# libshoal/Green-Marl

Measured on AMD Instinct MI355X. Metric: edges/s (GTEPS) per PageRank iter, RMAT-26, higher is better.
Workload: dtype f32; 1 GPU; pagerank RMAT-26 (V=67108864, E=1073741824), reference RMAT generator seed 1997 permute=1, d=0.85, fixed iterations; partition=1-D vertex, 1 rank(s), exchange=none, exchange_bytes_per_rank_and_step=0, exchange_packed=False, step_form=single rank, options=15

## Files before the change

### green-marl_amd/csrc/gmx_pr_cold.hip

```cpp
#pragma clang fp contract(off)

#include "gmx_internal.h"

#include <algorithm>
#include <rocprim/rocprim.hpp>

#define PRC_G 32
#define PRC_BLK_GROUPS 16
#define PRC_LDS_BYTES 131072
#define PRC_STAGE_BYTES 2048
#define PRC_LDS_LIMIT 163840
static constexpr int prc_tile_elems(int elem) { return (PRC_LDS_LIMIT - 16 * (PRC_STAGE_BYTES + 64 * elem) - 64) / elem; }
static constexpr int prc_tile_elems_classed(int elem) {
    return (PRC_LDS_LIMIT - 16 * 64 * elem - 64) / elem < 32768 ? (PRC_LDS_LIMIT - 16 * 64 * elem - 64) / elem / 8 * 8 : 32768;
}
#define PRC_THREADS 1024
#define PRC_WAVES (PRC_THREADS / 64)
#define PRC_UNROLL 4
#define PRC_PAD 0xffffu
#define PRC_END 0x8000u
#define PRC_Q1P 0
#define PRC_Q1E 64
#define PRC_Q2 128

#ifdef GMX_PR_BOUNDS
#define PRC_CHECK(cond) do { if (!(cond)) __builtin_trap(); } while (0)
#else
#define PRC_CHECK(cond) do { } while (0)
#endif

#define PRC_CLS_BITS 3
enum { PRC_CL_GEN = 0, PRC_CL_E1 = 1, PRC_CL_E2 = 2, PRC_CL_E4 = 3, PRC_CL_E8 = 4, PRC_CL_H = 5 };
enum { PRC_FORM_EDGE = 0, PRC_FORM_PAIR = 1, PRC_FORM_E1 = 2, PRC_FORM_E2 = 3, PRC_FORM_E4 = 4, PRC_FORM_E8 = 5, PRC_FORM_H = 6,
       PRC_FORM_TILE = 7 };
enum { PRC_TM_EDGE = 0, PRC_TM_PAIR = 1, PRC_TM_CLASSED = 2, PRC_TM_SINGLES = 3 };
__host__ __device__ static inline int prc_class_of_len(int len) { return len <= 1 ? PRC_CL_E1 : len == 2 ? PRC_CL_E2 : len <= 4 ? PRC_CL_E4 : len <= 8 ? PRC_CL_E8 : PRC_CL_H; }
__host__ __device__ static inline int prc_padded_len(int cls, int len) {
    return cls == PRC_CL_GEN ? len : cls == PRC_CL_H ? (len + 7) & ~7 : 1 << (cls - 1);
}

__host__ __device__ static inline int prc_e_stores(int L, int elem) { return ((8 / L) * elem + 15) / 16; }
__host__ __device__ static inline int64_t prc_interleaved_pos(int L, int elem, int64_t G, int i, int j) {
    const int K = prc_e_stores(L, elem), R = 16 / elem, cpg = K / 2;
    const int ch = i / (8 * R), within = i % (8 * R), m = within / R, r = within % R, q = (int) (G & 1) * cpg + ch;
    return (G & ~(int64_t) 1) * PRC_G + 8 * m + (q * R + r) * L + j;
}

struct prc_item1 { int32_t tile, g0, g1, form; };
struct prc_item2 { int32_t bin, g0, g1, slot; };
struct prc_item3 { int32_t bin, slot0, nslots, pad; };

struct pr_cold {
    pr_cold_params prm;
    int64_t Ec = 0;
    int64_t P1 = 0;
    int64_t P2 = 0;
    int64_t npairs = 0;
    int64_t ncold = 0;
    int tile = 0, binrows = 0, limbs = 1, lo_bits = 42;
    int64_t ntiles = 0, nbins = 0, ncells = 0;
    dbuf<uint16_t> srcl;
    dbuf<int32_t> ob;
    dbuf<uint16_t> rowl;
    dbuf<char> val;
    dbuf<char> cold;
    dbuf<prc_item1> it1p;
    dbuf<int32_t> torg;
    dbuf<int32_t> vstart;
    dbuf<prc_item2> it2;
    dbuf<prc_item3> it3;
    int64_t n1p = 0, n1e = 0, n2 = 0, n3 = 0, nslots = 0;
    std::vector<prc_item1> h1p, h1e;
    std::vector<prc_item2> h2;
    std::vector<prc_item3> h3;
    int nparts = 1;
    int64_t o1[3] = {0, 0, 0};
    int64_t o1g[2] = {0, 0};
    std::vector<int64_t> o2, o3, o3few;
    uint32_t q1 = 0, q1c = 0, q2 = 0;
    dbuf<unsigned long long> scratch;
    dbuf<unsigned int> queue;
    dbuf<double> diffp;
    int grid = 256;
    bool all_bins = false;
    std::vector<int32_t> tile_maxdeg;
};

static int prc_grid_for(int64_t n, int block = 256) {
    int64_t b = (n + block - 1) / block;
    if (b < 1) b = 1;
    if (b > 256 * 16) b = 256 * 16;
    return (int) b;
}

__global__ void prc_keys_kernel(const uint64_t* __restrict__ keys, int64_t n, pr_cold_params prm, int tile_src, int binrows,
                                int binbits, uint64_t* __restrict__ out) {
    int64_t i = (int64_t) blockIdx.x * blockDim.x + threadIdx.x;
    const int64_t stride = (int64_t) gridDim.x * blockDim.x;
    const int64_t span = prm.slice - prm.T;
    for (; i < n; i += stride) {
        const uint64_t k = keys[i];
        const int64_t row = (int64_t) (k >> 32) - prm.row_lo;
        const int64_t src = (int64_t) (uint32_t) k;
        const int64_t a = prm.index_of_row[row];
        const int64_t cp = (src / prm.slice) * span + (src % prm.slice - prm.T);
        const uint64_t t = (uint64_t) (cp / tile_src), sl = (uint64_t) (cp % tile_src);
        const uint64_t b = (uint64_t) (a / binrows), rl = (uint64_t) (a % binrows);
        out[i] = (t << (32 + binbits + PRC_CLS_BITS)) | (b << 32) | (rl << 16) | sl;
    }
}

__global__ void prc_runs_kernel(const uint64_t* __restrict__ k, int64_t n, const uint8_t* __restrict__ single, int tshift,
                                int32_t* __restrict__ cflag, int32_t* __restrict__ ps) {
    int64_t i = (int64_t) blockIdx.x * blockDim.x + threadIdx.x;
    const int64_t stride = (int64_t) gridDim.x * blockDim.x;
    for (; i < n; i += stride) {
        cflag[i] = (i == 0 || (k[i] >> 32) != (k[i - 1] >> 32)) ? 1 : 0;
        ps[i] = (i == 0 || (k[i] >> 16) != (k[i - 1] >> 16) || (single && single[k[i] >> tshift] == PRC_TM_SINGLES)) ? 1 : 0;
    }
}

__global__ void prc_pair_start_kernel(const int32_t* __restrict__ ps, const int32_t* __restrict__ pincl, int64_t n, int64_t np,
                                      int32_t* __restrict__ pstart) {
    int64_t i = (int64_t) blockIdx.x * blockDim.x + threadIdx.x;
    const int64_t stride = (int64_t) gridDim.x * blockDim.x;
    for (; i <= n; i += stride) {
        if (i == n) { pstart[np] = (int32_t) n; continue; }
        if (ps[i]) pstart[pincl[i] - 1] = (int32_t) i;
    }
}

__global__ void prc_tile_stats_kernel(const uint64_t* __restrict__ k, int64_t n, int shift, int64_t ntiles, const int32_t* __restrict__ pincl,
                                      const int32_t* __restrict__ cincl, int64_t np, int64_t nc, int32_t* __restrict__ out) {
    int64_t t = (int64_t) blockIdx.x * blockDim.x + threadIdx.x;
    const int64_t stride = (int64_t) gridDim.x * blockDim.x;
    for (; t <= ntiles; t += stride) {
        int64_t lo = 0, hi = n;
        while (lo < hi) {
            const int64_t mid = (lo + hi) >> 1;
            if ((int64_t) (k[mid] >> shift) < t) lo = mid + 1; else hi = mid;
        }
        out[3 * t + 0] = (int32_t) lo;
        out[3 * t + 1] = lo < n ? pincl[lo] - 1 : (int32_t) np;
        out[3 * t + 2] = lo < n ? cincl[lo] - 1 : (int32_t) nc;
    }
}

__global__ void prc_class_kernel(uint64_t* __restrict__ k, int64_t n, const int32_t* __restrict__ pincl, const int32_t* __restrict__ pstart,
                                 const uint8_t* __restrict__ mode, int binbits) {
    int64_t i = (int64_t) blockIdx.x * blockDim.x + threadIdx.x;
    const int64_t stride = (int64_t) gridDim.x * blockDim.x;
    for (; i < n; i += stride) {
        const uint64_t key = k[i];
        const int m = mode[key >> (32 + binbits + PRC_CLS_BITS)];
        if (m == PRC_TM_SINGLES) { k[i] = key | ((uint64_t) PRC_CL_E1 << (32 + binbits)); continue; }
        if (m != PRC_TM_CLASSED) continue;
        const int32_t p = pincl[i] - 1;
// ... 557 lines not shown

template <typename S, int FORM>
__device__ __forceinline__ void prc_class_block(const S* __restrict__ s_tile, S* __restrict__ stage, const prc_u32x4 cur, const int32_t o,
                                                S* __restrict__ val, const unsigned sink, const int lane) {
    if constexpr (FORM == PRC_FORM_H) prc_block_H<S>(s_tile, stage, cur, o, val, sink, lane);
    else prc_block_E<S, 1 << (FORM - PRC_FORM_E1)>(s_tile, cur, o, val, lane);
}

#define PRC_SET_WAIT_N(t, N)                                                                                        \
    asm volatile("s_waitcnt vmcnt(%8)"                                                                              \
                 : "+v"((t).e0), "+v"((t).e1), "+v"((t).e2), "+v"((t).e3), "+v"((t).o0), "+v"((t).o1), "+v"((t).o2), "+v"((t).o3) \
                 : "n"(N) : "memory")

template <typename S, int FORM>
__device__ __forceinline__ void prc_class_item(const prc_item1 d, const S* __restrict__ s_tile, S* __restrict__ stage,
                                               const uint16_t* __restrict__ srcl, const int32_t* __restrict__ ob,
                                               S* __restrict__ val, const unsigned sink, const int wv, const int lane) {
    constexpr int NST = prc_form_stores<S, FORM>::value;
    const int nblocks = (d.g1 - d.g0) / PRC_BLK_GROUPS;
    const int nsuper = nblocks / (PRC_WAVES * PRC_PAIR_DEPTH);
    const prc_u32x4* in = (const prc_u32x4*) srcl + ((int64_t) d.g0 * (PRC_G / 8) + wv * 64 + lane);
    const int32_t* obp = ob + (d.g0 + wv * PRC_BLK_GROUPS + (lane >> 2));
    constexpr int64_t IN_STEP = PRC_PAIR_DEPTH * PRC_WAVES * 64;
    constexpr int64_t OB_STEP = PRC_PAIR_DEPTH * PRC_WAVES * PRC_BLK_GROUPS;
    if (nsuper > 0) {
        prc_set A, B;
#define PRC_PROCESS(t)                                                                  \
    do {                                                                                \
        prc_class_block<S, FORM>(s_tile, stage, (t).e0, (t).o0, val, sink, lane);       \
        prc_class_block<S, FORM>(s_tile, stage, (t).e1, (t).o1, val, sink, lane);       \
        prc_class_block<S, FORM>(s_tile, stage, (t).e2, (t).o2, val, sink, lane);       \
        prc_class_block<S, FORM>(s_tile, stage, (t).e3, (t).o3, val, sink, lane);       \
    } while (0)
        prc_set_load(A, in, obp);
        {
            const int kn = 1 < nsuper ? 1 : 0;
            prc_set_load(B, in + kn * IN_STEP, obp + kn * OB_STEP);
        }
        PRC_SET_WAIT_N(A, 8);
        PRC_PROCESS(A);
        int k = 1;
#pragma unroll 1
        for (; k + 1 < nsuper; k += 2) {
            prc_set_load(A, in + (int64_t) (k + 1) * IN_STEP, obp + (int64_t) (k + 1) * OB_STEP);
            PRC_SET_WAIT_N(B, 4 * NST + 8);
            PRC_PROCESS(B);
            const int kn = k + 2 < nsuper ? k + 2 : k + 1;
            prc_set_load(B, in + (int64_t) kn * IN_STEP, obp + (int64_t) kn * OB_STEP);
            PRC_SET_WAIT_N(A, 4 * NST + 8);
            PRC_PROCESS(A);
        }
        PRC_SET_WAIT_N(B, 4 * NST);
        if (k < nsuper) PRC_PROCESS(B);
#undef PRC_PROCESS
    }
    {
        const int b0 = nsuper * (PRC_WAVES * PRC_PAIR_DEPTH);
        prc_u32x4 cur[PRC_PAIR_DEPTH];
        int32_t o[PRC_PAIR_DEPTH];
#pragma unroll
        for (int j = 0; j < PRC_PAIR_DEPTH; j++)
            if (b0 + j * PRC_WAVES + wv < nblocks) {
                const int64_t off = (int64_t) (b0 + j * PRC_WAVES);
                cur[j] = __builtin_nontemporal_load(in + off * 64);
                o[j] = __builtin_nontemporal_load(obp + off * PRC_BLK_GROUPS);
            }
#pragma unroll
        for (int j = 0; j < PRC_PAIR_DEPTH; j++)
            if (b0 + j * PRC_WAVES + wv < nblocks) prc_class_block<S, FORM>(s_tile, stage, cur[j], o[j], val, sink, lane);
    }
}

template <typename S>
__device__ __forceinline__ void prc_edge_item(const prc_item1 d, const S* __restrict__ s_tile,
                                              const uint16_t* __restrict__ srcl, const int32_t* __restrict__ ob,
                                              S* __restrict__ val, const int wv, const int lane) {
    typedef typename prc_vec4<S>::type V4;
    const int npieces = (d.g1 - d.g0 + 7) >> 3;
    for (int base = 0; base < npieces; base += PRC_WAVES * PRC_UNROLL) {
        prc_u32x2 ids[PRC_UNROLL];
        int32_t o[PRC_UNROLL];
#pragma unroll
        for (int u = 0; u < PRC_UNROLL; u++) {
            const int pc = base + u * PRC_WAVES + wv;
            const int g = d.g0 + pc * 8 + (lane >> 3);
            o[u] = -1;
            if (pc < npieces && g < d.g1) {
                ids[u] = __builtin_nontemporal_load((const prc_u32x2*) srcl + (int64_t) g * (PRC_G / 4) + (lane & 7));
                o[u] = __builtin_nontemporal_load(ob + g);
            }
        }
#pragma unroll
        for (int u = 0; u < PRC_UNROLL; u++) {
            if (o[u] < 0) continue;
            V4 v;
            v.x = s_tile[ids[u].x & 0x7fffu];
            v.y = s_tile[(ids[u].x >> 16) & 0x7fffu];
            v.z = s_tile[ids[u].y & 0x7fffu];
            v.w = s_tile[(ids[u].y >> 16) & 0x7fffu];
            __builtin_nontemporal_store(v, (V4*) (val + o[u]) + (lane & 7));
        }
    }
}

template <typename S, int TILE, bool CLASSED>
__global__ void __launch_bounds__(PRC_THREADS)
pr_cold_tile_kernel(const prc_item1* __restrict__ items, int n_items, unsigned int* __restrict__ queue,
                    const S* __restrict__ contrib, const int32_t* __restrict__ org, int nranks, int64_t span, int64_t slice, int64_t T,
                    const uint16_t* __restrict__ srcl, const int32_t* __restrict__ ob, S* __restrict__ val, unsigned sink_base,
                    unsigned qbase, const int32_t* __restrict__ vst) {
    __shared__ S s_tile[TILE];
    __shared__ S s_stage[PRC_WAVES][CLASSED ? 64 : PRC_STAGE_BYTES / sizeof(S) + 64];
    __shared__ int s_item;
    const int tid = threadIdx.x, lane = tid & 63;
    const int wv = __builtin_amdgcn_readfirstlane(tid >> 6);
    const unsigned sink = sink_base + (blockIdx.x * PRC_WAVES + wv) * 64 + lane;
    int loaded = -1;
    for (;;) {
        __syncthreads();
        if (tid == 0) s_item = (int) (atomicAdd(&queue[CLASSED ? PRC_Q1E : PRC_Q1P], 1u) - qbase);
        __syncthreads();
        const int it = s_item;
        if ((unsigned) it >= (unsigned) n_items) break;
        const prc_item1 d = items[it];
        if (d.tile != loaded) {
            prc_load_tile<S, TILE>(s_tile, d.tile, org, contrib, nranks, span, slice, T);
            loaded = d.tile;
            __syncthreads();
        }
        if constexpr (CLASSED) {
            const int32_t* vs = vst + ((int64_t) d.tile << PRC_CLS_BITS);
            for (int cls = PRC_CL_E1; cls <= PRC_CL_H; cls++) {
                const int32_t lo = max(d.g0, vs[cls]), hi = min(d.g1, vs[cls + 1]);
                if (lo >= hi) continue;
                const prc_item1 seg{d.tile, lo, hi, cls + 1};
                switch (cls) {
                case PRC_CL_E1: prc_class_item<S, PRC_FORM_E1>(seg, s_tile, s_stage[wv], srcl, ob, val, sink, wv, lane); break;
                case PRC_CL_E2: prc_class_item<S, PRC_FORM_E2>(seg, s_tile, s_stage[wv], srcl, ob, val, sink, wv, lane); break;
                case PRC_CL_E4: prc_class_item<S, PRC_FORM_E4>(seg, s_tile, s_stage[wv], srcl, ob, val, sink, wv, lane); break;
                case PRC_CL_E8: prc_class_item<S, PRC_FORM_E8>(seg, s_tile, s_stage[wv], srcl, ob, val, sink, wv, lane); break;
                default: prc_class_item<S, PRC_FORM_H>(seg, s_tile, s_stage[wv], srcl, ob, val, sink, wv, lane); break;
                }
            }
        } else {
            if (d.form == PRC_FORM_PAIR) prc_pair_item<S>(d, s_tile, s_stage[wv], srcl, ob, val, sink, wv, lane);
            else prc_edge_item<S>(d, s_tile, srcl, ob, val, wv, lane);
        }
    }
}

__device__ __forceinline__ unsigned long long prc_fix_hi(double v) { return (unsigned long long) (long long) (v * 0x1p62); }

template <typename S>
__device__ __forceinline__ void prc_finish_row(const pr_cold_fuse& fz, int64_t i, double sum, double& diff_acc) {
    const int32_t od = __builtin_nontemporal_load(fz.outdeg_c + i);
    const int64_t r = __builtin_nontemporal_load(fz.active + i);
    const double old = (double) __builtin_nontemporal_load((const S*) fz.rk_c + i);
    const S vs = (S) (fz.base + fz.d * sum);
    diff_acc += fabs((double) vs - old);
    __builtin_nontemporal_store(vs, (S*) fz.rk_c + i);
    __builtin_nontemporal_store(od > 0 ? (S) ((double) vs / (double) od) : (S) 0, (S*) fz.next_owned + r);
}

template <int THREADS>
__device__ __forceinline__ void prc_block_diff(double diff_acc, double* s_red, double* __restrict__ dst) {
#pragma unroll
    for (int off = 32; off > 0; off >>= 1) diff_acc += __shfl_down(diff_acc, off, 64);
    if ((threadIdx.x & 63) == 0) s_red[threadIdx.x >> 6] = diff_acc;
    __syncthreads();
    if (threadIdx.x == 0) {
        double t = 0.0;
#pragma unroll
        for (int w = 0; w < THREADS / 64; w++) t += s_red[w];
        *dst = t;
    }
}

template <typename S, int BINROWS, int LIMBS, bool FUSE>
__global__ void __launch_bounds__(PRC_THREADS)
pr_cold_accum_kernel(const prc_item2* __restrict__ items, int n_items, unsigned int* __restrict__ queue,
                     const uint16_t* __restrict__ rowl, const S* __restrict__ val, int64_t nactive, double lo_scale,
                     S* __restrict__ cold, unsigned long long* __restrict__ scratch, pr_cold_fuse fz,
                     double* __restrict__ diff_part, unsigned qbase) {
    typedef typename prc_vec4<S>::type V4;
    __shared__ unsigned long long s_acc[LIMBS * BINROWS];
    __shared__ double s_red[PRC_WAVES];
    __shared__ int s_item;
    const int tid = threadIdx.x, lane = tid & 63;
    const int wv = __builtin_amdgcn_readfirstlane(tid >> 6);
    for (;;) {
        __syncthreads();
        if (tid == 0) s_item = (int) (atomicAdd(&queue[PRC_Q2], 1u) - qbase);
#pragma unroll 4
        for (int i = tid; i < LIMBS * BINROWS; i += PRC_THREADS) s_acc[i] = 0ull;
        __syncthreads();
        const int it = s_item;
        if ((unsigned) it >= (unsigned) n_items) break;
        const prc_item2 d = items[it];
        const int npieces = (d.g1 - d.g0 + 7) >> 3;
        for (int base = 0; base < npieces; base += PRC_WAVES * PRC_UNROLL) {
            prc_u32x2 ids[PRC_UNROLL];
            V4 v[PRC_UNROLL];
            bool ok[PRC_UNROLL];
#pragma unroll
            for (int u = 0; u < PRC_UNROLL; u++) {
                const int pc = base + u * PRC_WAVES + wv;
                const int g = d.g0 + pc * 8 + (lane >> 3);
                ok[u] = pc < npieces && g < d.g1;
                if (ok[u]) {
                    const int64_t at = (int64_t) g * (PRC_G / 4) + (lane & 7);
                    ids[u] = __builtin_nontemporal_load((const prc_u32x2*) rowl + at);
                    v[u] = __builtin_nontemporal_load((const V4*) val + at);
                }
            }
#pragma unroll
            for (int u = 0; u < PRC_UNROLL; u++) {
                if (!ok[u]) continue;
                const unsigned r[4] = {ids[u].x & 0xffffu, ids[u].x >> 16, ids[u].y & 0xffffu, ids[u].y >> 16};
                const double x[4] = {(double) v[u].x, (double) v[u].y, (double) v[u].z, (double) v[u].w};
#pragma unroll
                for (int j = 0; j < 4; j++) {
                    if (r[j] == PRC_PAD) continue;
                    PRC_CHECK(r[j] < (unsigned) BINROWS && x[j] >= 0.0 && x[j] <= 1.0);
                    const unsigned long long hi = prc_fix_hi(x[j]);
                    __hip_atomic_fetch_add(&s_acc[r[j]], hi, __ATOMIC_RELAXED, __HIP_MEMORY_SCOPE_WORKGROUP);
                    if (LIMBS > 1) {
                        const double rem = x[j] - (double) (long long) hi * 0x1p-62;
                        const unsigned long long lo = (unsigned long long) (long long) (rem * 0x1p62 * lo_scale);
                        __hip_atomic_fetch_add(&s_acc[BINROWS + r[j]], lo, __ATOMIC_RELAXED, __HIP_MEMORY_SCOPE_WORKGROUP);
                    }
                }
            }
        }
        __syncthreads();
        double diff_acc = 0.0;
        if (d.slot < 0) {
            const int64_t i0 = (int64_t) d.bin * BINROWS;
#pragma unroll 4
            for (int r = tid; r < BINROWS; r += PRC_THREADS) {
                if (i0 + r >= nactive) break;
                double sum = (double) (long long) s_acc[r] * 0x1p-62;
                if (LIMBS > 1) sum += (double) (long long) s_acc[BINROWS + r] * (0x1p-62 / lo_scale);
                if (FUSE) prc_finish_row<S>(fz, i0 + r, sum, diff_acc);
                else __builtin_nontemporal_store((S) sum, cold + i0 + r);
            }
        } else {
            unsigned long long* dst = scratch + (int64_t) d.slot * (LIMBS * BINROWS);
#pragma unroll 4
            for (int i = tid; i < LIMBS * BINROWS; i += PRC_THREADS) dst[i] = s_acc[i];
        }
        if (FUSE) prc_block_diff<PRC_THREADS>(diff_acc, s_red, diff_part + it);
    }
}

template <typename S, int BINROWS, int LIMBS, bool FUSE>
__global__ void __launch_bounds__(1024)
pr_cold_reduce_kernel(const prc_item3* __restrict__ items, int64_t nactive, double lo_scale,
                      const unsigned long long* __restrict__ scratch, S* __restrict__ cold, pr_cold_fuse fz,
                      double* __restrict__ diff_part) {
    __shared__ unsigned long long s_part[LIMBS][16][64];
    const prc_item3 d = items[blockIdx.y];
    const int lane = threadIdx.x & 63, wv = threadIdx.x >> 6;
    const int r = blockIdx.x * 64 + lane;
    const int64_t i0 = (int64_t) d.bin * BINROWS;
    unsigned long long hi = 0, lo = 0;
    const unsigned long long* src = scratch + (int64_t) d.slot0 * (LIMBS * BINROWS) + r;
#pragma unroll 4
    for (int s = wv; s < d.nslots; s += 16) {
        hi += __builtin_nontemporal_load(src + (int64_t) s * (LIMBS * BINROWS));
        if (LIMBS > 1) lo += __builtin_nontemporal_load(src + (int64_t) s * (LIMBS * BINROWS) + BINROWS);
    }
    s_part[0][wv][lane] = hi;
    if (LIMBS > 1) s_part[LIMBS - 1][wv][lane] = lo;
    __syncthreads();
    if (wv == 0 && i0 + r < nactive) {
        hi = 0;
        lo = 0;
#pragma unroll
        for (int w = 0; w < 16; w++) {
            hi += s_part[0][w][lane];
            if (LIMBS > 1) lo += s_part[LIMBS - 1][w][lane];
        }
        double v = (double) (long long) hi * 0x1p-62;
        if (LIMBS > 1) v += (double) (long long) lo * (0x1p-62 / lo_scale);
        if (FUSE) {
            double diff_acc = 0.0;
            prc_finish_row<S>(fz, i0 + r, v, diff_acc);
            s_part[0][0][lane] = (unsigned long long) __double_as_longlong(diff_acc);
        } else cold[i0 + r] = (S) v;
    } else if (FUSE && wv == 0) s_part[0][0][lane] = 0ull;
    if (FUSE && wv == 0) {
        __builtin_amdgcn_wave_barrier();
        __builtin_amdgcn_s_waitcnt(0xc07f);
        __builtin_amdgcn_wave_barrier();
        if (lane == 0) {
            double t = 0.0;
            for (int l = 0; l < 64; l++) t += __longlong_as_double((long long) s_part[0][0][l]);
            diff_part[(int64_t) blockIdx.y * gridDim.x + blockIdx.x] = t;
        }
    }
}

#define PRC_FEW_SLOTS 8
template <typename S, int BINROWS, int LIMBS, bool FUSE>
__global__ void __launch_bounds__(256)
pr_cold_reduce_few_kernel(const prc_item3* __restrict__ items, int64_t nactive, double lo_scale,
                          const unsigned long long* __restrict__ scratch, S* __restrict__ cold, pr_cold_fuse fz,
                          double* __restrict__ diff_part) {
    const prc_item3 d = items[blockIdx.y];
    const int lane = threadIdx.x & 63;
    const int rg = blockIdx.x * 4 + (threadIdx.x >> 6);
    const int r = rg * 64 + lane;
    const int64_t i0 = (int64_t) d.bin * BINROWS;
    unsigned long long hi = 0, lo = 0;
    const unsigned long long* src = scratch + (int64_t) d.slot0 * (LIMBS * BINROWS) + r;
#pragma unroll 4
    for (int s = 0; s < d.nslots; s++) {
        hi += __builtin_nontemporal_load(src + (int64_t) s * (LIMBS * BINROWS));
        if (LIMBS > 1) lo += __builtin_nontemporal_load(src + (int64_t) s * (LIMBS * BINROWS) + BINROWS);
    }
    double diff_acc = 0.0;
    if (i0 + r < nactive) {
        double v = (double) (long long) hi * 0x1p-62;
        if (LIMBS > 1) v += (double) (long long) lo * (0x1p-62 / lo_scale);
        if (FUSE) prc_finish_row<S>(fz, i0 + r, v, diff_acc);
        else cold[i0 + r] = (S) v;
    }
    if (FUSE) {
        double t = 0.0;
        for (int l = 0; l < 64; l++) t += __shfl(diff_acc, l, 64);
        if (lane == 0) diff_part[(int64_t) blockIdx.y * (BINROWS / 64) + rg] = t;
    }
}

static int prc_upload_lists(pr_cold* c, const std::vector<uint8_t>* tile_class, const std::vector<int32_t>* bin_part, int nparts) {
    auto by_size1 = [](const prc_item1& a, const prc_item1& b) { return a.g1 - a.g0 > b.g1 - b.g0; };
    auto by_size2 = [](const prc_item2& a, const prc_item2& b) { return a.g1 - a.g0 > b.g1 - b.g0; };
    std::vector<prc_item1> l1;
    for (int k = 0; k < 2; k++) {
        c->o1[k] = (int64_t) l1.size();
        for (int part = 0; part < 3; part++) {
            if (part == 1) c->o1g[k] = (int64_t) l1.size();
            std::vector<prc_item1> a;
            for (const prc_item1& it : (part < 2 ? c->h1p : c->h1e))
                if ((tile_class ? (int) (*tile_class)[(size_t) it.tile] : 0) == k && (part == 2 || (part == 0) == (it.form >= PRC_FORM_E1))) a.push_back(it);
            std::stable_sort(a.begin(), a.end(), by_size1);
            l1.insert(l1.end(), a.begin(), a.end());
        }
    }
    c->o1[2] = (int64_t) l1.size();
    std::vector<prc_item2> l2;
    std::vector<prc_item3> l3;
    c->o2.assign((size_t) nparts + 1, 0);
    c->o3.assign((size_t) nparts + 1, 0);
    c->o3few.assign((size_t) nparts, 0);
    for (int q = 0; q < nparts; q++) {
        c->o2[(size_t) q] = (int64_t) l2.size();
        c->o3[(size_t) q] = (int64_t) l3.size();
        std::vector<prc_item2> a;
        for (const prc_item2& it : c->h2)
            if ((bin_part ? (*bin_part)[(size_t) it.bin] : 0) == q) a.push_back(it);
        std::stable_sort(a.begin(), a.end(), by_size2);
        l2.insert(l2.end(), a.begin(), a.end());
        for (int few = 1; few >= 0; few--)
            for (const prc_item3& it : c->h3)
                if ((bin_part ? (*bin_part)[(size_t) it.bin] : 0) == q && (it.nslots <= PRC_FEW_SLOTS ? 1 : 0) == few) {
                    l3.push_back(it);
                    if (few) c->o3few[(size_t) q]++;
                }
    }
    c->o2[(size_t) nparts] = (int64_t) l2.size();
    c->o3[(size_t) nparts] = (int64_t) l3.size();
    c->nparts = nparts;
    if ((int64_t) l1.size() != c->n1p + c->n1e || (int64_t) l2.size() != c->n2 || (int64_t) l3.size() != c->n3) {
        gmx_set_error("pr cold: work lists lost items while being regrouped");
        return GMX_ERR_ARG;
    }
    if (!l1.empty()) GMX_HIP(hipMemcpy(c->it1p.p, l1.data(), sizeof(prc_item1) * l1.size(), hipMemcpyHostToDevice));
    if (!l2.empty()) GMX_HIP(hipMemcpy(c->it2.p, l2.data(), sizeof(prc_item2) * l2.size(), hipMemcpyHostToDevice));
    if (!l3.empty()) GMX_HIP(hipMemcpy(c->it3.p, l3.data(), sizeof(prc_item3) * l3.size(), hipMemcpyHostToDevice));
    return GMX_OK;
}

int pr_cold_set_parts(pr_cold* c, int nparts, const int64_t* act_bound, int64_t hub, int64_t live) {
    if (!c || c->Ec == 0) return GMX_OK;
    if (nparts <= 1) return prc_upload_lists(c, nullptr, nullptr, 1);
    std::vector<int32_t> bin_part((size_t) c->nbins, 0);
    {
        std::vector<int64_t> bb((size_t) nparts + 1, 0);
        for (int j = 1; j < nparts; j++) bb[(size_t) j] = std::min<int64_t>(c->nbins, act_bound[j] / c->binrows);
        bb[(size_t) nparts] = c->nbins;
        for (int j = 0; j < nparts; j++)
            for (int64_t b = bb[(size_t) j]; b < bb[(size_t) j + 1]; b++) bin_part[(size_t) b] = nparts - 1 - j;
    }
    std::vector<uint8_t> tile_class((size_t) c->ntiles, 0);
    const int64_t span = c->prm.slice - c->prm.T, tile_src = c->tile - 1;
    for (int64_t t = 0; t < c->ntiles; t++) {
        const int64_t cp0 = t * tile_src, cp1 = std::min<int64_t>(cp0 + tile_src, span * c->prm.nranks);
        bool hub_only = true;
        for (int64_t r = cp0 / span; r * span < cp1 && hub_only; r++) {
            const int64_t o0 = c->prm.T + std::max<int64_t>(cp0, r * span) - r * span;
            const int64_t o1 = c->prm.T + std::min<int64_t>(cp1, (r + 1) * span) - r * span;
            if (o0 < live && std::min(o1, live) > hub) hub_only = false;
        }
// ... 517 lines not shown
```

Before: 748.9 GTEPS.

## Prefetch next work item and vectorize fused row finish in cold accumulate kernel

Restructures the cold accumulate kernel so the first batch of the next queue item is loaded while the current item's rows are finalized, and zeroes shared accumulators inline instead of in a separate pass. The row finish now reads outdegree and old rank as 4-wide vectors. The next-contribution values are staged in LDS so the scatter to next_owned is coalesced by lane. This aims to hide global load latency across item boundaries and cut per-row scalar memory traffic, at the cost of more registers and extra synchronization.

```diff
diff --git a/green-marl_amd/csrc/gmx_pr_cold.hip b/green-marl_amd/csrc/gmx_pr_cold.hip
--- a/green-marl_amd/csrc/gmx_pr_cold.hip
+++ b/green-marl_amd/csrc/gmx_pr_cold.hip
@@ -3,6 +3,7 @@
 #include "gmx_internal.h"
 
 #include <algorithm>
+#include <type_traits>
 #include <rocprim/rocprim.hpp>
 
 #define PRC_G 32
@@ -866,14 +867,19 @@
 __device__ __forceinline__ unsigned long long prc_fix_hi(double v) { return (unsigned long long) (long long) (v * 0x1p62); }
 
 template <typename S>
+__device__ __forceinline__ S prc_new_rank(const pr_cold_fuse& fz, double sum) { return (S) (fz.base + fz.d * sum); }
+template <typename S>
+__device__ __forceinline__ S prc_next_contrib(S vs, int32_t od) { return od > 0 ? (S) ((double) vs / (double) od) : (S) 0; }
+
+template <typename S>
 __device__ __forceinline__ void prc_finish_row(const pr_cold_fuse& fz, int64_t i, double sum, double& diff_acc) {
     const int32_t od = __builtin_nontemporal_load(fz.outdeg_c + i);
     const int64_t r = __builtin_nontemporal_load(fz.active + i);
     const double old = (double) __builtin_nontemporal_load((const S*) fz.rk_c + i);
-    const S vs = (S) (fz.base + fz.d * sum);
+    const S vs = prc_new_rank<S>(fz, sum);
     diff_acc += fabs((double) vs - old);
     __builtin_nontemporal_store(vs, (S*) fz.rk_c + i);
-    __builtin_nontemporal_store(od > 0 ? (S) ((double) vs / (double) od) : (S) 0, (S*) fz.next_owned + r);
+    __builtin_nontemporal_store(prc_next_contrib<S>(vs, od), (S*) fz.next_owned + r);
 }
 
 template <int THREADS>
@@ -888,6 +894,71 @@
         for (int w = 0; w < THREADS / 64; w++) t += s_red[w];
         *dst = t;
     }
+}
+
+#ifndef PRC_ACC_WIDE
+#define PRC_ACC_WIDE 0
+#endif
+#define PRC_ACC_ITEMS (PRC_ACC_WIDE ? 8 : 4)
+template <typename S, int U>
+struct prc_acc_batch {
+    typedef typename std::conditional<PRC_ACC_WIDE, prc_u32x4, prc_u32x2>::type ID;
+    ID ids[U];
+    typename prc_vec4<S>::type v[U][PRC_ACC_ITEMS / 4];
+    bool ok[U];
+};
+
+template <typename S, int U>
+__device__ __forceinline__ void prc_acc_load(prc_acc_batch<S, U>& b, const prc_item2& d, int base, int wv, int lane,
+                                             const uint16_t* __restrict__ rowl, const S* __restrict__ val) {
+    typedef typename prc_vec4<S>::type V4;
+    constexpr int LPG = PRC_G / PRC_ACC_ITEMS;
+#pragma unroll
+    for (int u = 0; u < U; u++) {
+        const int g = d.g0 + (base + u * PRC_WAVES + wv) * (64 / LPG) + lane / LPG;
+        b.ok[u] = g < d.g1;
+        if (b.ok[u]) {
+            const int64_t at = (int64_t) g * PRC_G + PRC_ACC_ITEMS * (lane % LPG);
+            b.ids[u] = __builtin_nontemporal_load((const typename prc_acc_batch<S, U>::ID*) (rowl + at));
+#pragma unroll
+            for (int k = 0; k < PRC_ACC_ITEMS / 4; k++) b.v[u][k] = __builtin_nontemporal_load((const V4*) (val + at) + k);
+        }
+    }
+}
+
+template <typename S, int BINROWS, int LIMBS, int U>
+__device__ __forceinline__ void prc_acc_add(unsigned long long* s_acc, const prc_acc_batch<S, U>& b, double lo_scale) {
+#pragma unroll
+    for (int u = 0; u < U; u++) {
+        if (!b.ok[u]) continue;
+#pragma unroll
+        for (int j = 0; j < PRC_ACC_ITEMS; j++) {
+            const unsigned r = (b.ids[u][j >> 1] >> (16 * (j & 1))) & 0xffffu;
+            if (r == PRC_PAD) continue;
+            const double x = (double) b.v[u][j >> 2][j & 3];
+            PRC_CHECK(r < (unsigned) BINROWS && x >= 0.0 && x <= 1.0);
+            const unsigned long long hi = prc_fix_hi(x);
+            __hip_atomic_fetch_add(&s_acc[r], hi, __ATOMIC_RELAXED, __HIP_MEMORY_SCOPE_WORKGROUP);
+            if (LIMBS > 1) {
+                const double rem = x - (double) (long long) hi * 0x1p-62;
+                const unsigned long long lo = (unsigned long long) (long long) (rem * 0x1p62 * lo_scale);
+                __hip_atomic_fetch_add(&s_acc[BINROWS + r], lo, __ATOMIC_RELAXED, __HIP_MEMORY_SCOPE_WORKGROUP);
+            }
+        }
+    }
+}
+
+__device__ __forceinline__ unsigned long long prc_bits(float v) { return __float_as_uint(v); }
+__device__ __forceinline__ unsigned long long prc_bits(double v) { return (unsigned long long) __double_as_longlong(v); }
+template <typename S> __device__ __forceinline__ S prc_from_bits(unsigned long long w);
+template <> __device__ __forceinline__ float prc_from_bits<float>(unsigned long long w) { return __uint_as_float((unsigned) w); }
+template <> __device__ __forceinline__ double prc_from_bits<double>(unsigned long long w) { return __longlong_as_double((long long) w); }
+
+template <int LIMBS>
+__device__ __forceinline__ double prc_row_sum(unsigned long long hi, unsigned long long lo, double lo_scale) {
+    double sum = (double) (long long) hi * 0x1p-62;
+    if (LIMBS > 1) sum += (double) (long long) lo * (0x1p-62 / lo_scale);
+    return sum;
 }
 
 template <typename S, int BINROWS, int LIMBS, bool FUSE>
@@ -897,73 +968,141 @@
                      S* __restrict__ cold, unsigned long long* __restrict__ scratch, pr_cold_fuse fz,
                      double* __restrict__ diff_part, unsigned qbase) {
     typedef typename prc_vec4<S>::type V4;
-    __shared__ unsigned long long s_acc[LIMBS * BINROWS];
+    typedef int prc_i32x4 __attribute__((ext_vector_type(4)));
+    typedef unsigned long long prc_u64x2 __attribute__((ext_vector_type(2)));
+    constexpr int U = PRC_ACC_WIDE ? PRC_UNROLL / 2 : PRC_UNROLL;
+    constexpr int GPP = 64 * PRC_ACC_ITEMS / PRC_G;
+    constexpr int NQ = BINROWS / 4 / PRC_THREADS;
+    static_assert(BINROWS % (4 * PRC_THREADS) == 0, "whole rounds of 4 rows");
+    __shared__ __attribute__((aligned(16))) unsigned long long s_acc[LIMBS * BINROWS];
     __shared__ double s_red[PRC_WAVES];
     __shared__ int s_item;
     const int tid = threadIdx.x, lane = tid & 63;
     const int wv = __builtin_amdgcn_readfirstlane(tid >> 6);
-    for (;;) {
+#pragma unroll 4
+    for (int i = tid; i < LIMBS * BINROWS; i += PRC_THREADS) s_acc[i] = 0ull;
+    if (tid == 0) s_item = (int) (atomicAdd(&queue[PRC_Q2], 1u) - qbase);
+    __syncthreads();
+    int it = s_item;
+    prc_item2 d{};
+    prc_acc_batch<S, U> b;
+    if ((unsigned) it < (unsigned) n_items) {
+        d = items[it];
+        prc_acc_load<S, U>(b, d, 0, wv, lane, rowl, val);
+    }
+    while ((unsigned) it < (unsigned) n_items) {
+        const int npieces = (d.g1 - d.g0 + GPP - 1) / GPP;
+        prc_acc_add<S, BINROWS, LIMBS, U>(s_acc, b, lo_scale);
+        for (int base = PRC_WAVES * U; base < npieces; base += PRC_WAVES * U) {
+            prc_acc_load<S, U>(b, d, base, wv, lane, rowl, val);
+            prc_acc_add<S, BINROWS, LIMBS, U>(s_acc, b, lo_scale);
+        }
+        if (tid == 0) s_item = (int) (atomicAdd(&queue[PRC_Q2], 1u) - qbase);
         __syncthreads();
-        if (tid == 0) s_item = (int) (atomicAdd(&queue[PRC_Q2], 1u) - qbase);
-#pragma unroll 4
-        for (int i = tid; i < LIMBS * BINROWS; i += PRC_THREADS) s_acc[i] = 0ull;
-        __syncthreads();
-        const int it = s_item;
-        if ((unsigned) it >= (unsigned) n_items) break;
-        const prc_item2 d = items[it];
-        const int npieces = (d.g1 - d.g0 + 7) >> 3;
-        for (int base = 0; base < npieces; base += PRC_WAVES * PRC_UNROLL) {
-            prc_u32x2 ids[PRC_UNROLL];
-            V4 v[PRC_UNROLL];
-            bool ok[PRC_UNROLL];
-#pragma unroll
-            for (int u = 0; u < PRC_UNROLL; u++) {
-                const int pc = base + u * PRC_WAVES + wv;
-                const int g = d.g0 + pc * 8 + (lane >> 3);
-                ok[u] = pc < npieces && g < d.g1;
-                if (ok[u]) {
-                    const int64_t at = (int64_t) g * (PRC_G / 4) + (lane & 7);
-                    ids[u] = __builtin_nontemporal_load((const prc_u32x2*) rowl + at);
-                    v[u] = __builtin_nontemporal_load((const V4*) val + at);
+        const int nit = s_item;
+        prc_item2 nd{};
+        if ((unsigned) nit < (unsigned) n_items) {
+            nd = items[nit];
+            prc_acc_load<S, U>(b, nd, 0, wv, lane, rowl, val);
+        }
+        double diff_acc = 0.0;
+        if (d.slot < 0) {
+            const int64_t i0 = (int64_t) d.bin * BINROWS;
+            prc_i32x4 od[NQ];
+            V4 old[NQ];
+            bool full[NQ];
+#pragma unroll
+            for (int q = 0; q < NQ; q++) {
+                const int64_t i = i0 + 4 * (q * PRC_THREADS + tid);
+                full[q] = i + 4 <= nactive;
+                if (FUSE && full[q]) {
+                    od[q] = __builtin_nontemporal_load((const prc_i32x4*) (fz.outdeg_c + i));
+                    old[q] = __builtin_nontemporal_load((const V4*) ((const S*) fz.rk_c + i));
                 }
             }
 #pragma unroll
-            for (int u = 0; u < PRC_UNROLL; u++) {
-                if (!ok[u]) continue;
-                const unsigned r[4] = {ids[u].x & 0xffffu, ids[u].x >> 16, ids[u].y & 0xffffu, ids[u].y >> 16};
-                const double x[4] = {(double) v[u].x, (double) v[u].y, (double) v[u].z, (double) v[u].w};
-#pragma unroll
-                for (int j = 0; j < 4; j++) {
-                    if (r[j] == PRC_PAD) continue;
-                    PRC_CHECK(r[j] < (unsigned) BINROWS && x[j] >= 0.0 && x[j] <= 1.0);
-                    const unsigned long long hi = prc_fix_hi(x[j]);
-                    __hip_atomic_fetch_add(&s_acc[r[j]], hi, __ATOMIC_RELAXED, __HIP_MEMORY_SCOPE_WORKGROUP);
+            for (int q = 0; q < NQ; q++) {
+                const int r = 4 * (q * PRC_THREADS + tid);
+                const int64_t i = i0 + r;
+                prc_u64x2* a = (prc_u64x2*) (s_acc + r);
+                prc_u64x2* al = (prc_u64x2*) (s_acc + (LIMBS - 1) * BINROWS + r);
+                const prc_u64x2 h0 = a[0], h1 = a[1];
+                prc_u64x2 l0{0ull, 0ull}, l1{0ull, 0ull};
+                if (LIMBS > 1) {
+                    l0 = al[0];
+                    l1 = al[1];
+                }
+                const double sum[4] = {prc_row_sum<LIMBS>(h0.x, l0.x, lo_scale), prc_row_sum<LIMBS>(h0.y, l0.y, lo_scale),
+                                       prc_row_sum<LIMBS>(h1.x, l1.x, lo_scale), prc_row_sum<LIMBS>(h1.y, l1.y, lo_scale)};
+                if (FUSE && full[q]) {
+                    const S vs[4] = {prc_new_rank<S>(fz, sum[0]), prc_new_rank<S>(fz, sum[1]),
+                                     prc_new_rank<S>(fz, sum[2]), prc_new_rank<S>(fz, sum[3])};
+                    diff_acc += fabs((double) vs[0] - (double) old[q].x);
+                    diff_acc += fabs((double) vs[1] - (double) old[q].y);
+                    diff_acc += fabs((double) vs[2] - (double) old[q].z);
+                    diff_acc += fabs((double) vs[3] - (double) old[q].w);
+                    __builtin_nontemporal_store(V4{vs[0], vs[1], vs[2], vs[3]}, (V4*) ((S*) fz.rk_c + i));
+                    const S nv[4] = {prc_next_contrib<S>(vs[0], od[q].x), prc_next_contrib<S>(vs[1], od[q].y),
+                                     prc_next_contrib<S>(vs[2], od[q].z), prc_next_contrib<S>(vs[3], od[q].w)};
+                    a[0] = prc_u64x2{prc_bits(nv[0]), prc_bits(nv[1])};
+                    a[1] = prc_u64x2{prc_bits(nv[2]), prc_bits(nv[3])};
                     if (LIMBS > 1) {
-                        const double rem = x[j] - (double) (long long) hi * 0x1p-62;
-                        const unsigned long long lo = (unsigned long long) (long long) (rem * 0x1p62 * lo_scale);
-                        __hip_atomic_fetch_add(&s_acc[BINROWS + r[j]], lo, __ATOMIC_RELAXED, __HIP_MEMORY_SCOPE_WORKGROUP);
+                        al[0] = prc_u64x2{0ull, 0ull};
+                        al[1] = prc_u64x2{0ull, 0ull};
+                    }
+                } else {
+                    a[0] = prc_u64x2{0ull, 0ull};
+                    a[1] = prc_u64x2{0ull, 0ull};
+                    if (LIMBS > 1) {
+                        al[0] = prc_u64x2{0ull, 0ull};
+                        al[1] = prc_u64x2{0ull, 0ull};
+                    }
+                    if (!FUSE && full[q]) {
+                        __builtin_nontemporal_store(V4{(S) sum[0], (S) sum[1], (S) sum[2], (S) sum[3]}, (V4*) (cold + i));
+                    } else {
+#pragma unroll
+                        for (int j = 0; j < 4; j++) {
+                            if (i + j >= nactive) break;
+                            if (FUSE) prc_finish_row<S>(fz, i + j, sum[j], diff_acc);
+                            else __builtin_nontemporal_store((S) sum[j], cold + i + j);
+                        }
                     }
                 }
             }
-        }
-        __syncthreads();
-        double diff_acc = 0.0;
-        if (d.slot < 0) {
-            const int64_t i0 = (int64_t) d.bin * BINROWS;
-#pragma unroll 4
-            for (int r = tid; r < BINROWS; r += PRC_THREADS) {
-                if (i0 + r >= nactive) break;
-                double sum = (double) (long long) s_acc[r] * 0x1p-62;
-                if (LIMBS > 1) sum += (double) (long long) s_acc[BINROWS + r] * (0x1p-62 / lo_scale);
-                if (FUSE) prc_finish_row<S>(fz, i0 + r, sum, diff_acc);
-                else __builtin_nontemporal_store((S) sum, cold + i0 + r);
+            if (FUSE) {
+                __syncthreads();
+                S* nx = (S*) fz.next_owned;
+#pragma unroll 1
+                for (int q = 0; q < NQ; q++) {
+                    int32_t at[4];
+#pragma unroll
+                    for (int j = 0; j < 4; j++) {
+                        const int rr = 4 * (q * PRC_THREADS + wv * 64) + 64 * j + lane;
+                        at[j] = i0 + (rr & ~3) + 4 <= nactive ? __builtin_nontemporal_load(fz.active + i0 + rr) : -1;
+                    }
+#pragma unroll
+                    for (int j = 0; j < 4; j++) {
+                        if (at[j] < 0) continue;
+                        const int rr = 4 * (q * PRC_THREADS + wv * 64) + 64 * j + lane;
+                        const unsigned long long w = s_acc[rr];
+                        s_acc[rr] = 0ull;
+                        __builtin_nontemporal_store(prc_from_bits<S>(w), nx + at[j]);
+                    }
+                }
             }
         } else {
-            unsigned long long* dst = scratch + (int64_t) d.slot * (LIMBS * BINROWS);
+            prc_u64x2* dst = (prc_u64x2*) (scratch + (int64_t) d.slot * (LIMBS * BINROWS));
+            prc_u64x2* src = (prc_u64x2*) s_acc;
 #pragma unroll 4
-            for (int i = tid; i < LIMBS * BINROWS; i += PRC_THREADS) dst[i] = s_acc[i];
+            for (int i = tid; i < LIMBS * BINROWS / 2; i += PRC_THREADS) {
+                dst[i] = src[i];
+                src[i] = prc_u64x2{0ull, 0ull};
+            }
         }
         if (FUSE) prc_block_diff<PRC_THREADS>(diff_acc, s_red, diff_part + it);
+        __syncthreads();
+        it = nit;
+        d = nd;
     }
 }
 
```

New measurement: 748.6 GTEPS (median of 2 runs). About the same (-0.0%).
